# eigenkernel/eigenkernel

Measured on AMD Instinct MI355X. Metric: eigenpairs/s (full spectrum) + achieved fp64 TFLOP/s vs roofline, N=16384 GEP, higher is better.
Workload: dtype f64

## Files before the change

### eigenkernel_amd/csrc/ek_sb2st.hip

```cpp
#include "ek_common.h"
#include "ek_switch.h"

#include <cstdlib>
#include <type_traits>
#include <vector>

namespace ek {
namespace {

typedef double double4_t __attribute__((ext_vector_type(4)));

constexpr int SB = kBandW;
constexpr int LDAB = 2 * SB;
constexpr int DLD = SB + 1;

__device__ __forceinline__ double ld_sc1(const double *p) {
  return __longlong_as_double((long long)__hip_atomic_load((const unsigned long long *)p, __ATOMIC_RELAXED,
                                                           __HIP_MEMORY_SCOPE_AGENT));
}
__device__ __forceinline__ void st_sc1(double *p, double v) {
  __hip_atomic_store((unsigned long long *)p, (unsigned long long)__double_as_longlong(v), __ATOMIC_RELAXED,
                     __HIP_MEMORY_SCOPE_AGENT);
}
template <int CTRL>
__device__ __forceinline__ double dpp_mov(double v) {
  const int lo = __builtin_amdgcn_update_dpp(0, __double2loint(v), CTRL, 0xf, 0xf, false);
  const int hi = __builtin_amdgcn_update_dpp(0, __double2hiint(v), CTRL, 0xf, 0xf, false);
  return __hiloint2double(hi, lo);
}
template <int W>
__device__ __forceinline__ double group_sum(double v) {
  if (W >= 2) v += dpp_mov<0xB1>(v);
  if (W >= 4) v += dpp_mov<0x4E>(v);
  if (W >= 8) v += dpp_mov<0x141>(v);
  if (W >= 16) v += dpp_mov<0x140>(v);
  return v;
}
__device__ __forceinline__ double lane_value(double v, int l) {
  const int lo = __builtin_amdgcn_readlane(__double2loint(v), l);
  const int hi = __builtin_amdgcn_readlane(__double2hiint(v), l);
  return __hiloint2double(hi, lo);
}
template <int CTRL, int ROWMASK>
__device__ __forceinline__ double dpp_mov_rows(double v) {
  const int lo = __builtin_amdgcn_update_dpp(0, __double2loint(v), CTRL, ROWMASK, 0xf, false);
  const int hi = __builtin_amdgcn_update_dpp(0, __double2hiint(v), CTRL, ROWMASK, 0xf, false);
  return __hiloint2double(hi, lo);
}
__device__ __forceinline__ double wave_sum(double v) {
  v = group_sum<16>(v);
  v += dpp_mov_rows<0x142, 0xA>(v);
  v += dpp_mov_rows<0x143, 0xC>(v);
  return lane_value(v, 63);
}
__device__ __forceinline__ void wave_sync() {
  __builtin_amdgcn_s_waitcnt(0xc07f);
  __builtin_amdgcn_wave_barrier();
}

__global__ void pack_band_kernel(int n, const double *__restrict__ A, int lda, double *__restrict__ AB) {
  const int c = blockIdx.x;
  for (int d = threadIdx.x; d < LDAB; d += blockDim.x) {
    double v = 0.0;
    if (d <= SB && c + d < n) v = A[(size_t)(c + d) + (size_t)c * lda];
    AB[(size_t)d + (size_t)c * LDAB] = v;
  }
}
__global__ void unpack_de_kernel(int n, const double *__restrict__ AB, double *__restrict__ d, double *__restrict__ e) {
  const int c = blockIdx.x * blockDim.x + threadIdx.x;
  if (c >= n) return;
  d[c] = AB[(size_t)c * LDAB];
  if (c < n - 1) e[c] = AB[1 + (size_t)c * LDAB];
}

struct ChaseArgs {
  int n, nsweeps;
  double *AB;
  double *V2; int ldv2;
  double *tau2; int ldt;
  unsigned *prog;
  unsigned *ctl;
  double *mail; int kmax;
  int only_if_abandoned;
  const int *skip;
};

constexpr unsigned kSpinLimit = 1u << 22;

struct Reflector { double v, tau, beta; };

__device__ __forceinline__ Reflector reflector_of(double x, int lane) {
#pragma clang fp contract(off)
  const double ssq = wave_sum((lane >= 1) ? x * x : 0.0);
  const double alpha0 = lane_value(x, 0);
  Reflector r;
  r.beta = alpha0; r.tau = 0.0;
  double scale = 0.0;
  const double nrm2 = __builtin_fma(alpha0, alpha0, ssq);
  if (ssq != 0.0 && nrm2 > 1e-290) {
    r.beta = -copysign(sqrt(nrm2), alpha0);
    r.tau = (r.beta - alpha0) / r.beta;
    scale = 1.0 / (alpha0 - r.beta);
  }
  r.v = (lane == 0) ? 1.0 : x * scale;
  return r;
}
template <int CW>
__device__ __forceinline__ void task_partials(const double (&dd)[CW], const double (&bk)[CW], const double (&vc)[CW],
                                              double &pp, double &qq) {
#pragma clang fp contract(off)
  pp = 0.0; qq = 0.0;
#pragma unroll
  for (int j = 0; j < CW; ++j) { pp = __builtin_fma(dd[j], vc[j], pp); qq = __builtin_fma(bk[j], vc[j], qq); }
}
__device__ __forceinline__ double task_col0(double bk0, double tau, double qs, double vc0) {
#pragma clang fp contract(off)
  const double t = tau * qs;
  return __builtin_fma(-t, vc0, bk0);
}
__device__ __forceinline__ double task_w(double tau, double psum, double v_r) {
#pragma clang fp contract(off)
  const double p_r = tau * psum;
  const double dot = wave_sum(p_r * v_r);
  const double alpha = (-0.5 * tau) * dot;
  return __builtin_fma(alpha, v_r, p_r);
}
__device__ __forceinline__ double task_rank2(double d, double v_r, double w_c, double w_r, double v_c) {
#pragma clang fp contract(off)
  const double t1 = v_r * w_c, t2 = w_r * v_c;
  return d - (t1 + t2);
}
__device__ __forceinline__ double task_right(double b, double q_r, double v_c) {
#pragma clang fp contract(off)
  return __builtin_fma(-q_r, v_c, b);
}
template <int CW>
__device__ __forceinline__ void task_left(double (&bp)[CW], double vn_r, double tau_n, double *st, int lane, bool skip0) {
#pragma clang fp contract(off)
  constexpr int LPC = 64 / CW;
#pragma unroll
  for (int j = 0; j < CW; ++j) st[j * 65 + lane] = vn_r * bp[j];
  wave_sync();
  double tot_b;
  {
    const int j = lane / LPC, q = lane % LPC;
    const double *src = st + j * 65 + CW * q;
    double a0 = 0.0, a1 = 0.0;
#pragma unroll
    for (int l = 0; l < CW; l += 2) { a0 += src[l]; a1 += src[l + 1]; }
    tot_b = group_sum<LPC>(a0 + a1);
  }
  const double u = tau_n * vn_r;
#pragma unroll
  for (int j = 0; j < CW; ++j)
    if (!(skip0 && j == 0)) bp[j] = __builtin_fma(-u, lane_value(tot_b, j * LPC), bp[j]);
  wave_sync();
}

constexpr int MAILW = 72;
constexpr unsigned long long kMailEmpty = 0x7ff8dead0000beefull;

__device__ __forceinline__ bool mail_empty(double v) { return (unsigned long long)__double_as_longlong(v) == kMailEmpty; }

__global__ void mail_init_kernel(double *mail, int count) {
  const int i = blockIdx.x * blockDim.x + threadIdx.x;
  if (i < count) mail[i] = __longlong_as_double((long long)kMailEmpty);
}

template <int NW>
__global__ __launch_bounds__(64 * NW) void chase_kernel(ChaseArgs p) {
  constexpr int CW = SB / NW;
  __shared__ __attribute__((aligned(16))) double s_v[2][SB];
  __shared__ double s_p[NW][SB], s_q[NW][SB];
  __shared__ double s_t[NW][CW * 65];
  __shared__ double s_D[SB * DLD];
  __shared__ double s_tau[2];
  __shared__ int s_sweep, s_ok;
  const int t = threadIdx.x, lane = t & 63, wave = t >> 6;
  const int n = p.n;
  const int c0w = CW * wave;
  double *AB = p.AB;
  if (p.only_if_abandoned && !__hip_atomic_load(&p.ctl[3], __ATOMIC_RELAXED, __HIP_MEMORY_SCOPE_AGENT)) return;
  if (p.skip && (*p.skip & 0xff)) return;
  if (t == 0) s_ok = 1;
  auto give_up = [&]() { __hip_atomic_store(&p.ctl[1], 1u, __ATOMIC_RELAXED, __HIP_MEMORY_SCOPE_AGENT); };
  auto wait_word = [&](const unsigned *w, unsigned need) -> bool {
    unsigned spins = 0;
    while (__hip_atomic_load(w, __ATOMIC_RELAXED, __HIP_MEMORY_SCOPE_AGENT) < need) {
      __builtin_amdgcn_s_sleep(1);
      if ((++spins & 63u) == 0u &&
          (spins > kSpinLimit || __hip_atomic_load(&p.ctl[1], __ATOMIC_RELAXED, __HIP_MEMORY_SCOPE_AGENT)))
        return false;
    }
    return true;
  };
  auto put_reflector = [&](const Reflector &r, int L, int i0, int s, int k, double *sv, double *stau) {
    sv[lane] = r.v;
    if (lane == 0) { *stau = r.tau; p.tau2[(size_t)k + (size_t)s * p.ldt] = r.tau; }
    if (lane < L) p.V2[(size_t)(i0 + lane) + (size_t)s * p.ldv2] = r.v;
  };
  while (true) {
    __syncthreads();
    if (t == 0) s_sweep = (int)atomicAdd(&p.ctl[0], 1u);
    __syncthreads();
    const int s = s_sweep;
    if (s >= p.nsweeps) break;
    const int K = (n - 3 - s) / SB + 1;
    const int Kprev = (s > 0) ? (n - 2 - s) / SB + 1 : 0;
    const bool has_follower = s + 1 < p.nsweeps;
    for (int k = 0; k < K; ++k) {
      const int i0 = s + 1 + k * SB;
      const int L = (n - i0 < SB) ? n - i0 : SB;
      int L1 = n - i0 - SB; if (L1 > SB) L1 = SB; if (L1 < 0) L1 = 0;
      const bool lead = s > 0 && k + 1 < Kprev;
      double *mail = p.mail + ((size_t)((s - 1) & 3) * p.kmax + (k + 1)) * MAILW;
      if (t == 0 && s > 0) {
        if (!wait_word(&p.prog[s - 1], (unsigned)(k + 1 < Kprev ? k + 1 : Kprev))) { give_up(); s_ok = 0; }
      }
      __syncthreads();
      if (!s_ok) return;
      double dl[CW], bk[CW];
#pragma unroll
      for (int j = 0; j < CW; ++j) {
        const int c = c0w + j;
        dl[j] = (lane < L && c <= lane) ? ld_sc1(AB + (unsigned)((lane - c) + (i0 + c) * LDAB)) : 0.0;
        bk[j] = (lane < L1 && c < L) ? ld_sc1(AB + (unsigned)((SB + lane - c) + (i0 + c) * LDAB)) : 0.0;
      }
      double m_a = 0.0, m_b = 0.0;
      if (lead && wave == NW - 1) {
        m_a = ld_sc1(mail + ((lane < 63) ? lane + 1 : 64));
        if (lane == 63) m_b = ld_sc1(mail);
      }
      const int cur = k & 1;
      if (k == 0) {
        if (wave == 0) {
          const double x = (lane < L) ? ld_sc1(AB + (size_t)(1 + lane) + (size_t)s * LDAB) : 0.0;
          const Reflector r = reflector_of(x, lane);
          put_reflector(r, L, i0, s, k, s_v[cur], &s_tau[cur]);
          if (lane < L) st_sc1(AB + (size_t)(1 + lane) + (size_t)s * LDAB, (lane == 0) ? r.beta : 0.0);
        }
        __syncthreads();
      }
      const double tau = s_tau[cur];
      const double v_r = s_v[cur][lane];
      double vc[CW];
#pragma unroll
      for (int j = 0; j < CW; ++j) vc[j] = s_v[cur][c0w + j];
      if (lead && wave == NW - 1) {
        unsigned spins = 0;
        bool ok = true;
        while (__any(mail_empty(m_a) || (lane == 63 && mail_empty(m_b)))) {
          if ((++spins & 63u) == 0u &&
              (spins > kSpinLimit || __hip_atomic_load(&p.ctl[1], __ATOMIC_RELAXED, __HIP_MEMORY_SCOPE_AGENT))) {
            ok = false; break;
          }
          __builtin_amdgcn_s_sleep(1);
          if (mail_empty(m_a)) m_a = ld_sc1(mail + ((lane < 63) ? lane + 1 : 64));
          if (lane == 63 && mail_empty(m_b)) m_b = ld_sc1(mail);
        }
        if (!ok) { if (lane == 0) { give_up(); s_ok = 0; } }
        else {
          bk[CW - 1] = (lane < L1 && SB - 1 < L) ? m_a : 0.0;
          if (lane == 63 && SB - 1 < L) dl[CW - 1] = m_b;
          const double e = __longlong_as_double((long long)kMailEmpty);
          st_sc1(mail + ((lane < 63) ? lane + 1 : 64), e);
          if (lane == 63) st_sc1(mail, e);
        }
      }
#pragma unroll
      for (int j = 0; j < CW; ++j) {
        const int c = c0w + j;
        if (c <= lane) { s_D[lane * DLD + c] = dl[j]; s_D[c * DLD + lane] = dl[j]; }
      }
      __syncthreads();
      if (!s_ok) return;
      double dd[CW];
      {
        double pp, qq;
#pragma unroll
        for (int j = 0; j < CW; ++j) dd[j] = s_D[lane * DLD + c0w + j];
        task_partials<CW>(dd, bk, vc, pp, qq);
        s_p[wave][lane] = pp; s_q[wave][lane] = qq;
      }
      __syncthreads();
      if (wave == 0) {
        double qs = 0.0;
#pragma unroll
        for (int w = 0; w < NW; ++w) qs += s_q[w][lane];
        const double col0 = (L1 > 0) ? task_col0(bk[0], tau, qs, vc[0]) : 0.0;
        double b00 = col0;
        if (k + 1 < K) {
          const int i0n = i0 + SB;
          const Reflector r = reflector_of(col0, lane);
          put_reflector(r, L1, i0n, s, k + 1, s_v[cur ^ 1], &s_tau[cur ^ 1]);
          b00 = r.beta;
          if (lane < L1 && !(lane == 0 && k > 0 && has_follower))
            st_sc1(AB + (unsigned)((SB + lane) + i0 * LDAB), (lane == 0) ? r.beta : 0.0);
        }
        if (lane == 0 && k > 0 && has_follower)
          st_sc1(p.mail + ((size_t)(s & 3) * p.kmax + k) * MAILW + 64, b00);
      }
      double psum = 0.0;
#pragma unroll
      for (int w = 0; w < NW; ++w) psum += s_p[w][lane];
      const double w_r = task_w(tau, psum, v_r);
#pragma unroll
      for (int j = 0; j < CW; ++j) {
        const int c = c0w + j;
        dd[j] = task_rank2(dd[j], v_r, lane_value(w_r, c), w_r, vc[j]);
        if (c == 0 && k > 0 && has_follower)
          st_sc1(p.mail + ((size_t)(s & 3) * p.kmax + k) * MAILW + lane, dd[j]);
        if (c <= lane && lane < L && !(c == 0 && k > 0 && has_follower))
          st_sc1(AB + (unsigned)((lane - c) + (i0 + c) * LDAB), dd[j]);
      }
      double bp[CW];
#pragma unroll
      for (int j = 0; j < CW; ++j) bp[j] = 0.0;
      if (L1 > 0) {
        double qsum = 0.0;
#pragma unroll
        for (int w = 0; w < NW; ++w) qsum += s_q[w][lane];
        const double q_r = tau * qsum;
#pragma unroll
        for (int j = 0; j < CW; ++j) bp[j] = task_right(bk[j], q_r, vc[j]);
        if (k == K - 1) {
#pragma unroll
          for (int j = 0; j < CW; ++j) {
            const int c = c0w + j;
            if (lane < L1 && c < L && !(lane == 0 && c == 0 && k > 0 && has_follower))
              st_sc1(AB + (unsigned)((SB + lane - c) + (i0 + c) * LDAB), bp[j]);
          }
        }
      }
      if (k + 1 < K) {
        __syncthreads();
        task_left<CW>(bp, s_v[cur ^ 1][lane], s_tau[cur ^ 1], s_t[wave], lane, wave == 0);
#pragma unroll
        for (int j = 0; j < CW; ++j) {
          const int c = c0w + j;
          if (c > 0 && lane < L1)
            st_sc1(AB + (unsigned)((SB + lane - c) + (i0 + c) * LDAB), bp[j]);
        }
        asm volatile("s_waitcnt vmcnt(0)" ::: "memory");
        __syncthreads();
        if (t == 0) __hip_atomic_store(&p.prog[s], (unsigned)(k + 1), __ATOMIC_RELAXED, __HIP_MEMORY_SCOPE_AGENT);
      }
    }
    asm volatile("s_waitcnt vmcnt(0)" ::: "memory");
    __syncthreads();
    if (t == 0) __hip_atomic_store(&p.prog[s], (unsigned)K, __ATOMIC_RELAXED, __HIP_MEMORY_SCOPE_AGENT);
  }
}

constexpr int PMAILW = 80;
struct PosArgs {
  int n, K0;
  double *AB;
  double *V2; int ldv2;
  double *tau2; int ldt;
  double *fwd, *bwd;
  unsigned *retired;
  unsigned *ctl;
  unsigned census_spins;
  const int *skip;
  unsigned jitter;
};

template <int CTRL>
__device__ __forceinline__ double dpp_shift(double v) {
  const int lo = __builtin_amdgcn_update_dpp(__double2loint(v), __double2loint(v), CTRL, 0xf, 0xf, false);
  const int hi = __builtin_amdgcn_update_dpp(__double2hiint(v), __double2hiint(v), CTRL, 0xf, 0xf, false);
  return __hiloint2double(hi, lo);
}

__global__ __launch_bounds__(512) void chase_pos_kernel(PosArgs p) {
  constexpr int NW = 8, CW = SB / NW;
  __shared__ __attribute__((aligned(16))) double s_v[2][SB];
  __shared__ double s_p[NW][SB], s_q[NW][SB];
  __shared__ double s_t[NW][CW * 65];
  __shared__ double s_x[NW][SB], s_y[NW][SB], s_row[SB], s_b0[SB];
  __shared__ double s_tau[2], s_b00;
  __shared__ int s_ok;
  constexpr int RW = 1;
  const int t = threadIdx.x, lane = t & 63, wave = t >> 6;
  const int k = (int)blockIdx.x;
  if (k >= p.K0) return;
  if (p.skip && (*p.skip & 0xff)) return;
  const int n = p.n;
  const int c0w = CW * wave;
  double *AB = p.AB;
  unsigned *abandoned = &p.ctl[3];
  auto give_up = [&]() { __hip_atomic_store(abandoned, 1u, __ATOMIC_RELAXED, __HIP_MEMORY_SCOPE_AGENT); };
  if (t == 0) {
    int ok = 1;
    atomicAdd(&p.ctl[4], 1u);
    unsigned spins = 0;
    while (__hip_atomic_load(&p.ctl[4], __ATOMIC_RELAXED, __HIP_MEMORY_SCOPE_AGENT) < (unsigned)p.K0) {
      __builtin_amdgcn_s_sleep(8);
      if (++spins > p.census_spins || __hip_atomic_load(abandoned, __ATOMIC_RELAXED, __HIP_MEMORY_SCOPE_AGENT)) { ok = 0; break; }
    }
    if (!ok) give_up();
    s_ok = ok;
  }
  __syncthreads();
  if (!s_ok) return;
  auto take_line = [&](double *line, bool with65, double &a, double &b) -> bool {
    const bool l65 = with65 && lane == 0;
    a = ld_sc1(line + lane); b = l65 ? ld_sc1(line + 64) : 0.0;
    __builtin_amdgcn_s_sleep(2);
    double a2 = ld_sc1(line + lane), b2 = l65 ? ld_sc1(line + 64) : 0.0;
    unsigned spins = 0;
    while (__any(mail_empty(a) || (l65 && mail_empty(b)))) {
      if ((++spins & 63u) == 0u &&
          (spins > kSpinLimit || __hip_atomic_load(abandoned, __ATOMIC_RELAXED, __HIP_MEMORY_SCOPE_AGENT)))
        return false;
      a = a2; b = b2;
      a2 = ld_sc1(line + lane); b2 = l65 ? ld_sc1(line + 64) : 0.0;
    }
    const double e = __longlong_as_double((long long)kMailEmpty);
    st_sc1(line + lane, e);
    if (l65) st_sc1(line + 64, e);
    return true;
  };
  const int s_last = n - 3 - SB * k;
  double dd[CW], bk[CW];
  {
    const int i0 = 1 + SB * k;
    const int L = (n - i0 < SB) ? n - i0 : SB;
    int L1 = n - i0 - SB; if (L1 > SB) L1 = SB; if (L1 < 0) L1 = 0;
#pragma unroll
    for (int j = 0; j < CW; ++j) {
      const int c = c0w + j;
      const int hi = (lane > c) ? lane : c, lo = (lane > c) ? c : lane;
      dd[j] = (lane < L && c < L) ? AB[(size_t)(hi - lo) + (size_t)(i0 + lo) * LDAB] : 0.0;
      bk[j] = (lane < L1 && c < L) ? AB[(size_t)(SB + lane - c) + (size_t)(i0 + c) * LDAB] : 0.0;
    }
  }
  double xnext = 0.0;
  for (int s = 0; s <= s_last; ++s) {
    const int i0 = s + 1 + k * SB;
    const int L = (n - i0 < SB) ? n - i0 : SB;
    int L1 = n - i0 - SB; if (L1 > SB) L1 = SB; if (L1 < 0) L1 = 0;
    const int K = (n - 3 - s) / SB + 1;
    const int Kprev = (s > 0) ? (n - 2 - s) / SB + 1 : 0;
    const bool lead = s > 0 && k + 1 < Kprev;
    asm volatile("s_waitcnt vmcnt(0)" ::: "memory");
    if (p.jitter) {
      const unsigned h = ((unsigned)s * 2654435761u) ^ ((unsigned)k * 40503u * p.jitter);
      if (((h >> 9) & 15u) == 0u) for (unsigned q = 0; q < ((h >> 3) & 63u); ++q) __builtin_amdgcn_s_sleep(64);
    }
    if (wave == 0) {
      if (k == 0) {
        const double x = (s == 0) ? ((lane < L) ? AB[(size_t)(1 + lane)] : 0.0) : xnext;
        const Reflector r = reflector_of(x, lane);
        s_v[0][lane] = r.v;
        if (lane == 0) { s_tau[0] = r.tau; p.tau2[(size_t)s * p.ldt] = r.tau; AB[(size_t)1 + (size_t)s * LDAB] = r.beta; }
        if (lane < L) p.V2[(size_t)(i0 + lane) + (size_t)s * p.ldv2] = r.v;
      } else {
        double a, b;
        if (!take_line(p.fwd + ((size_t)k * 4 + (s & 3)) * PMAILW, false, a, b)) { if (lane == 0) { give_up(); s_ok = 0; } }
        s_v[0][lane] = (lane == 0) ? 1.0 : a;
        if (lane == 0) s_tau[0] = a;
      }
    }
    if (wave == NW - 1 && s > 0) {
      if (lead) {
        double a, b;
        if (!take_line(p.bwd + ((size_t)k * 4 + ((s - 1) & 3)) * PMAILW, true, a, b)) { if (lane == 0) { give_up(); s_ok = 0; } }
        const double up = dpp_shift<0x130>(a);
        const double beta = lane_value(b, 0), corner = lane_value(a, 0);
        const double col = (lane < 63) ? up : beta;
        bk[CW - 1] = (lane < L1 && SB - 1 < L) ? col : 0.0;
        if (lane == 63 && SB - 1 < L) dd[CW - 1] = corner;
      } else if (L == SB) {
        int ok = 1;
        if (lane == 0) {
          unsigned spins = 0;
          while (!__hip_atomic_load(&p.retired[k + 1], __ATOMIC_RELAXED, __HIP_MEMORY_SCOPE_AGENT)) {
            __builtin_amdgcn_s_sleep(1);
            if ((++spins & 63u) == 0u &&
                (spins > kSpinLimit || __hip_atomic_load(abandoned, __ATOMIC_RELAXED, __HIP_MEMORY_SCOPE_AGENT))) { ok = 0; break; }
          }
          if (!ok) { give_up(); s_ok = 0; }
        }
        wave_sync();
        const double corner = ld_sc1(AB + (size_t)(i0 + SB - 1) * LDAB);
        if (lane == 63) dd[CW - 1] = corner;
      }
    }
    __syncthreads();
    if (!s_ok) return;
    const double tau = s_tau[0];
    const double v_r = s_v[0][lane];
    double vc[CW];
#pragma unroll
    for (int j = 0; j < CW; ++j) vc[j] = s_v[0][c0w + j];
    {
      double pp, qq;
      task_partials<CW>(dd, bk, vc, pp, qq);
      s_p[wave][lane] = pp; s_q[wave][lane] = qq;
      if (wave == 0) s_b0[lane] = bk[0];
    }
    __syncthreads();
    if (wave == RW) {
      double qs = 0.0;
#pragma unroll
      for (int w = 0; w < NW; ++w) qs += s_q[w][lane];
      const double col0 = (L1 > 0) ? task_col0(s_b0[lane], tau, qs, s_v[0][0]) : 0.0;
      double b00 = col0;
      if (k + 1 < K) {
        const Reflector r = reflector_of(col0, lane);
        double *line = p.fwd + ((size_t)(k + 1) * 4 + (s & 3)) * PMAILW;
        st_sc1(line + lane, (lane == 0) ? r.tau : r.v);
        s_v[1][lane] = r.v;
        if (lane == 0) { s_tau[1] = r.tau; p.tau2[(size_t)(k + 1) + (size_t)s * p.ldt] = r.tau; }
        if (lane < L1) p.V2[(size_t)(i0 + SB + lane) + (size_t)s * p.ldv2] = r.v;
        b00 = r.beta;
      }
      if (lane == 0) {
        if (k > 0) st_sc1(p.bwd + ((size_t)(k - 1) * 4 + (s & 3)) * PMAILW + 64, b00);
        else s_b00 = b00;
      }
    }
    double psum = 0.0;
#pragma unroll
    for (int w = 0; w < NW; ++w) psum += s_p[w][lane];
    const double w_r = task_w(tau, psum, v_r);
    if (wave == 0) {
      dd[0] = task_rank2(dd[0], v_r, lane_value(w_r, 0), w_r, vc[0]);
      if (k > 0) st_sc1(p.bwd + ((size_t)(k - 1) * 4 + (s & 3)) * PMAILW + lane, dd[0]);
      else if (lane == 0) AB[(size_t)(s + 1) * LDAB] = dd[0];
    }
#pragma unroll
    for (int j = 0; j < CW; ++j)
      if (!(wave == 0 && j == 0)) dd[j] = task_rank2(dd[j], v_r, lane_value(w_r, c0w + j), w_r, vc[j]);
    double bp[CW];
    {
      double qsum = 0.0;
#pragma unroll
      for (int w = 0; w < NW; ++w) qsum += s_q[w][lane];
      const double q_r = tau * qsum;
#pragma unroll
      for (int j = 0; j < CW; ++j) bp[j] = (L1 > 0) ? task_right(bk[j], q_r, vc[j]) : 0.0;
    }
    if (k + 1 < K) {
      __syncthreads();
      task_left<CW>(bp, s_v[1][lane], s_tau[1], s_t[wave], lane, wave == 0);
    }
    if (s == s_last) break;
    if (lane == 0) {
#pragma unroll
      for (int j = 0; j < CW; ++j) s_row[c0w + j] = bp[j];
    }
    s_x[wave][lane] = dd[0]; s_y[wave][lane] = bp[0];
    __syncthreads();
    if (k == 0 && wave == 0) {
      const double up = dpp_shift<0x130>(dd[0]);
      xnext = (lane < 63) ? up : s_b00;
    }
#pragma unroll
    for (int j = 0; j + 1 < CW; ++j) { dd[j] = dd[j + 1]; bk[j] = bp[j + 1]; }
    dd[CW - 1] = (wave + 1 < NW) ? s_x[(wave + 1) & (NW - 1)][lane] : 0.0;
    bk[CW - 1] = (wave + 1 < NW) ? s_y[(wave + 1) & (NW - 1)][lane] : 0.0;
#pragma unroll
    for (int j = 0; j < CW; ++j) {
      const double brow0 = lane_value(bk[j], 0);
      const double du = dpp_shift<0x130>(dd[j]), bu = dpp_shift<0x130>(bk[j]);
      dd[j] = (lane == 63) ? brow0 : du;
      bk[j] = (lane == 63) ? 0.0 : bu;
    }
    if (wave == NW - 1) dd[CW - 1] = (lane < 63) ? s_row[lane + 1] : 0.0;
  }
  if (wave == 0) {
    if (lane == 1) {
      st_sc1(AB + (size_t)(n - 1) * LDAB, dd[1]);
      if (k == 0) st_sc1(AB + (size_t)1 + (size_t)(n - 2) * LDAB, dd[0]);
    }
    asm volatile("s_waitcnt vmcnt(0)" ::: "memory");
    if (lane == 0) __hip_atomic_store(&p.retired[k], 1u, __ATOMIC_RELAXED, __HIP_MEMORY_SCOPE_AGENT);
  }
}

__global__ void set_word_kernel(unsigned *p, unsigned v) { *p = v; }

__global__ void repack_band_kernel(int n, const double *__restrict__ AB0, double *__restrict__ AB, const unsigned *ctl) {
  if (!ctl[3]) return;
  const int c = blockIdx.x;
  for (int d = threadIdx.x; d < LDAB; d += blockDim.x) AB[(size_t)d + (size_t)c * LDAB] = AB0[(size_t)d + (size_t)c * LDAB];
}

constexpr int QG = 32;
constexpr int QR = QG + SB;
constexpr int QVLD = QG + 1;
constexpr int QREC = 2 * QR * QG;

struct Q2Geom {
  int n, nsweeps, nS, kmax;
  const unsigned *offS;
};
__host__ __device__ inline int q2_first_sweep(int S) { return S * QG - 1; }
__host__ __device__ inline int q2_groups_of_block(int n, int S) {
  int s0 = q2_first_sweep(S); if (s0 < 0) s0 = 0;
  return (s0 <= n - 3) ? (n - 3 - s0) / SB + 1 : 0;
}

__device__ __forceinline__ double q2_v_entry(const Q2Geom &g, const double *__restrict__ V2, int ldv2, int S, int k,
                                             int rr, int i) {
  const int s = q2_first_sweep(S) + i, o = S * QG + k * SB, row = o + rr;
  if (s < 0 || s >= g.nsweeps || rr < i || rr >= i + SB || row >= g.n) return 0.0;
  if (s + 1 + k * SB > g.n - 2) return 0.0;
  return V2[(size_t)row + (size_t)s * ldv2];
}

__global__ __launch_bounds__(256) void q2_tfactor_kernel(Q2Geom g, const double *__restrict__ V2, int ldv2,
                                                         const double *__restrict__ tau2, int ldt,
                                                         double *__restrict__ Rec) {
  __shared__ double sV[QR * QVLD];
  __shared__ double sG[QG * QVLD];
  __shared__ double sT[QG * QVLD];
  __shared__ double s_tau[QG];
  const int S = blockIdx.y, k = blockIdx.x, t = threadIdx.x, lane = t & 63, wave = t >> 6;
  const int l15 = lane & 15, l4 = lane >> 4;
  if (k >= q2_groups_of_block(g.n, S)) return;
  double *rec = Rec + ((size_t)g.offS[S] + k) * QREC;
  for (int idx = t; idx < QR * QG; idx += 256) {
    const int rr = idx % QR, i = idx / QR;
    const double v = q2_v_entry(g, V2, ldv2, S, k, rr, i);
    sV[rr * QVLD + i] = v;
    rec[rr * QG + i] = v;
  }
  for (int idx = t; idx < QG * QVLD; idx += 256) sT[idx] = 0.0;
  if (t < QG) {
    const int s = q2_first_sweep(S) + t;
    const bool exists = s >= 0 && s < g.nsweeps && s + 1 + k * SB <= g.n - 2;
    s_tau[t] = exists ? tau2[(size_t)k + (size_t)s * ldt] : 0.0;
  }
  __syncthreads();
  {
    const int ti = wave >> 1, tj = wave & 1;
    double4_t acc = (double4_t){0.0, 0.0, 0.0, 0.0};
    for (int kk = 0; kk < QR; kk += 4) {
      const double x = sV[(kk + l4) * QVLD + 16 * ti + l15];
      const double y = sV[(kk + l4) * QVLD + 16 * tj + l15];
      acc = __builtin_amdgcn_mfma_f64_16x16x4f64(x, y, acc, 0, 0, 0);
    }
#pragma unroll
    for (int r = 0; r < 4; ++r) sG[(16 * ti + l4 + 4 * r) * QVLD + 16 * tj + l15] = acc[r];
  }
  __syncthreads();
  if (wave == 0) {
    for (int i = 0; i < QG; ++i) {
      const double ti = s_tau[i];
      if (lane < i) {
        double a0 = 0.0, a1 = 0.0;
        int l = lane;
        for (; l + 1 < i; l += 2) {
          a0 += sT[lane * QVLD + l] * sG[l * QVLD + i];
          a1 += sT[lane * QVLD + l + 1] * sG[(l + 1) * QVLD + i];
        }
        if (l < i) a0 += sT[lane * QVLD + l] * sG[l * QVLD + i];
        sT[lane * QVLD + i] = -ti * (a0 + a1);
      } else if (lane == i) sT[i * QVLD + i] = ti;
      wave_sync();
    }
  }
  __syncthreads();
  for (int tile = wave; tile < 12; tile += 4) {
    const int ti = tile >> 1, tj = tile & 1;
    double4_t acc = (double4_t){0.0, 0.0, 0.0, 0.0};
#pragma unroll
    for (int kk = 0; kk < QG; kk += 4) {
      const double x = sV[(16 * ti + l15) * QVLD + kk + l4];
      const double y = sT[(kk + l4) * QVLD + 16 * tj + l15];
      acc = __builtin_amdgcn_mfma_f64_16x16x4f64(x, y, acc, 0, 0, 0);
    }
#pragma unroll
    for (int r = 0; r < 4; ++r) rec[QR * QG + (16 * ti + l4 + 4 * r) * QG + 16 * tj + l15] = -acc[r];
  }
}

constexpr int QNC = 64;
constexpr int QSTLD = 34;
constexpr int QVS = QG, QTS = QG + 2;
constexpr int QOPSZ = QR * QVS + QR * QTS;
constexpr unsigned kQ2Done = 0x7fffffffu;

struct Q2ApplyArgs {
  Q2Geom g;
  const double *Rec;
  double *Z; int ldz; int ncols;
  int nslab, npass, npair;
  unsigned *prog;
  unsigned *ctl;
};

typedef double d2_t __attribute__((ext_vector_type(2)));
__device__ __forceinline__ void st_sc1_x2(double *p, double a, double b) {
  d2_t v = {a, b};
  asm volatile("global_store_dwordx4 %0, %1, off sc1" :: "v"(p), "v"(v) : "memory");
}

#ifndef Q2_PF
#define Q2_PF 1
#endif
#ifndef Q2_PUTV0
#define Q2_PUTV0 24
#define Q2_PUTVS 4
#endif
template <int NBLK>
__global__ __launch_bounds__(256, 2) void q2_apply_nb_kernel(Q2ApplyArgs p) {
  constexpr int WT = 2 * NBLK + 4;
  extern __shared__ __attribute__((aligned(16))) double q2smem[];
  double *sOp = q2smem;
  __shared__ int s_pass, s_ok;
  const int t = threadIdx.x, lane = t & 63, wave = t >> 6, l15 = lane & 15, l4 = lane >> 4;
  double *st = q2smem + QOPSZ + wave * 16 * QSTLD;
  const int n = p.g.n;
  const double *sV = sOp, *sVT = sOp + QR * QVS;
  while (true) {
    __syncthreads();
    if (t == 0) s_pass = (int)atomicAdd(&p.ctl[2], 1u);
    __syncthreads();
    const int pass = __builtin_amdgcn_readfirstlane(s_pass);
    if (pass >= p.npass) break;
    const int bundle = p.npair - 1 - pass / p.nslab, slab = pass % p.nslab;
    const int S = NBLK * bundle;
    auto ks_of = [&](int b) -> int { return (S + b < p.g.nS) ? q2_groups_of_block(n, S + b) : 0; };
    auto off_of = [&](int b) -> unsigned {
      return (S + b < p.g.nS) ? (unsigned)__builtin_amdgcn_readfirstlane((int)p.g.offS[S + b]) : 0u;
    };
    const int KS0 = ks_of(0), KS1 = NBLK > 1 ? ks_of(1) : 0, KS2 = NBLK > 2 ? ks_of(2) : 0, KS3 = NBLK > 3 ? ks_of(3) : 0;
    const unsigned of0 = off_of(0), of1 = NBLK > 1 ? off_of(1) : 0u, of2 = NBLK > 2 ? off_of(2) : 0u, of3 = NBLK > 3 ? off_of(3) : 0u;
    auto KSb = [&](int b) -> int { return b == 0 ? KS0 : (b == 1 ? KS1 : (b == 2 ? KS2 : KS3)); };
    const int KS = KS0;
    const int colw = slab * QNC + 16 * wave;
    const unsigned *pprog = (bundle + 1 < p.npair) ? p.prog + (size_t)(pass - p.nslab) : nullptr;
    unsigned *myprog = p.prog + pass;
    if (KS <= 0) { if (t == 0) __hip_atomic_store(myprog, kQ2Done, __ATOMIC_RELAXED, __HIP_MEMORY_SCOPE_AGENT); continue; }
    const int o0 = S * QG;
    auto wait_for = [&](unsigned need) -> bool {
      if (!pprog) return true;
      unsigned spins = 0;
      while (__hip_atomic_load(pprog, __ATOMIC_RELAXED, __HIP_MEMORY_SCOPE_AGENT) < need) {
        __builtin_amdgcn_s_sleep(2);
        if ((++spins & 63u) == 0u &&
            (spins > kSpinLimit || __hip_atomic_load(&p.ctl[1], __ATOMIC_RELAXED, __HIP_MEMORY_SCOPE_AGENT)))
          return false;
      }
      return true;
    };
    double4_t w[WT];
    static_assert(QR * QG == 6 * 256 * 2, "a half record is six 16-byte pairs per thread");
    constexpr int HALF = QR * QG / 2;
    double zreg[16];
    d2_t oreg[12];
    const int obase_v = (t >> 4) * QVS + ((2 * (t & 15) + 16 * ((t >> 4) & 1)) & 31);
    const int obase_t = (t >> 4) * QTS + 2 * (t & 15);
    const int vsw = 16 * (l4 & 1);
    auto rec_of = [&](int b, int k) -> const d2_t * {
      const unsigned o = b == 0 ? of0 : (b == 1 ? of1 : (b == 2 ? of2 : of3));
      return reinterpret_cast<const d2_t *>(p.Rec + ((size_t)o + k) * QREC) + t;
    };
    auto fetch_v = [&](const d2_t *rec) {
#pragma unroll
      for (int q = 0; q < 6; ++q) oreg[q] = rec[256 * q];
    };
    auto fetch_t = [&](const d2_t *rec) {
#pragma unroll
      for (int q = 0; q < 6; ++q) oreg[6 + q] = rec[HALF + 256 * q];
    };
    auto put_v = [&](int q) { *reinterpret_cast<d2_t *>(sOp + obase_v + q * 16 * QVS) = oreg[q]; };
    auto put_t = [&](int q) { *reinterpret_cast<d2_t *>(sOp + QR * QVS + obase_t + q * 16 * QTS) = oreg[6 + q]; };
    const bool cols_in = colw + 16 <= p.ncols;
    auto fetch_rows = [&](int row0) {
      const int row = row0 + lane;
      const double *src = p.Z + (size_t)row + (size_t)colw * p.ldz;
      if (cols_in && row0 + SB <= n) {
#pragma unroll
        for (int c = 0; c < 16; ++c) zreg[c] = ld_sc1(src + (size_t)c * p.ldz);
      } else {
#pragma unroll
        for (int c = 0; c < 16; ++c)
          zreg[c] = (row < n && colw + c < p.ncols) ? ld_sc1(src + (size_t)c * p.ldz) : 0.0;
      }
    };
    auto half_to_tiles = [&](int h, double4_t &ta, double4_t &tb) {
      if ((lane >> 5) == h) {
#pragma unroll
        for (int c = 0; c < 16; ++c) st[c * QSTLD + (lane & 31)] = zreg[c];
      }
      wave_sync();
#pragma unroll
      for (int r = 0; r < 4; ++r) { ta[r] = st[l15 * QSTLD + l4 + 4 * r]; tb[r] = st[l15 * QSTLD + 16 + l4 + 4 * r]; }
      wave_sync();
    };
    auto tiles_to_rows = [&](int row0, const double4_t &ta, const double4_t &tb) {
#pragma unroll
      for (int r = 0; r < 4; ++r) { st[l15 * QSTLD + l4 + 4 * r] = ta[r]; st[l15 * QSTLD + 16 + l4 + 4 * r] = tb[r]; }
      wave_sync();
      {
        const int pr = lane & 15, cg = lane >> 4;
        const int row = row0 + 2 * pr;
        double *dst0 = p.Z + (size_t)row + (size_t)(colw + 4 * cg) * p.ldz;
        if (cols_in && row0 + 32 <= n) {
#pragma unroll
          for (int q = 0; q < 4; ++q) {
            const int c = 4 * cg + q;
            st_sc1_x2(dst0 + (size_t)q * p.ldz, st[c * QSTLD + 2 * pr], st[c * QSTLD + 2 * pr + 1]);
          }
        } else {
#pragma unroll
          for (int q = 0; q < 4; ++q) {
            const int c = 4 * cg + q;
            if (colw + c < p.ncols) {
              const double a = st[c * QSTLD + 2 * pr], b = st[c * QSTLD + 2 * pr + 1];
              if (row + 1 < n) st_sc1_x2(dst0 + (size_t)q * p.ldz, a, b);
              else if (row < n) st_sc1(dst0 + (size_t)q * p.ldz, a);
            }
          }
        }
      }
      wave_sync();
    };
    auto apply_group = [&](auto off_c, const d2_t *nrec, int row_next) {
      constexpr int OFF = decltype(off_c)::value;
      constexpr int PF = Q2_PF;
      double4_t w1[2];
      w1[0] = (double4_t){0.0, 0.0, 0.0, 0.0}; w1[1] = (double4_t){0.0, 0.0, 0.0, 0.0};
      {
        double pa[PF + 1][2];
        auto ld1 = [&](int sidx, int slot) {
          const double *vrow = sV + (16 * (sidx >> 2) + 4 * (sidx & 3) + l4) * QVS + l15;
          pa[slot][0] = vrow[vsw]; pa[slot][1] = vrow[16 - vsw];
        };
#pragma unroll
        for (int q = 0; q < PF; ++q) ld1(q, q);
#pragma unroll
        for (int sidx = 0; sidx < 24; ++sidx) {
          if (sidx + PF < 24) ld1(sidx + PF, (sidx + PF) % (PF + 1));
          if (sidx < 12 && (sidx & 1) == 0) put_t(sidx >> 1);
          if (sidx == 12) {
            fetch_v(nrec);
            if (row_next >= 0) fetch_rows(row_next);
          }
          const int tile = sidx >> 2, r = sidx & 3;
          const double y = w[tile + OFF][r];
          if (tile < 5) w1[0] = __builtin_amdgcn_mfma_f64_16x16x4f64(pa[sidx % (PF + 1)][0], y, w1[0], 0, 0, 0);
          if (tile > 0) w1[1] = __builtin_amdgcn_mfma_f64_16x16x4f64(pa[sidx % (PF + 1)][1], y, w1[1], 0, 0, 0);
        }
      }
      __syncthreads();
      fetch_t(nrec);
      {
        double px[PF + 1];
        auto seq_tile = [](int q) { return 2 * (q >> 4) + (q & 1); };
        auto seq_kk = [](int q) { return 4 * ((q & 15) >> 1); };
        auto seq_ok = [&](int q) { return !(seq_tile(q) == 5 && seq_kk(q) < 16); };
        auto ld2 = [&](int q, int slot) {
          if (seq_ok(q)) px[slot] = sVT[(16 * seq_tile(q) + l15) * QTS + l4 + seq_kk(q)];
        };
#pragma unroll
        for (int q = 0; q < PF; ++q) ld2(q, q);
#pragma unroll
        for (int q = 0; q < 48; ++q) {
          if (q + PF < 48) ld2(q + PF, (q + PF) % (PF + 1));
          if (q >= Q2_PUTV0 && q < Q2_PUTV0 + 6 * Q2_PUTVS && (q - Q2_PUTV0) % Q2_PUTVS == 0) put_v((q - Q2_PUTV0) / Q2_PUTVS);
          if (seq_ok(q)) {
            const int tile = seq_tile(q), kk = seq_kk(q);
            w[tile + OFF] = __builtin_amdgcn_mfma_f64_16x16x4f64(px[q % (PF + 1)], w1[kk >> 4][(kk & 15) >> 2], w[tile + OFF], 0, 0, 0);
          }
        }
      }
    };
    auto first_block = [&](int k) -> int {
      int b = 0;
#pragma unroll
      for (int q = 1; q < NBLK; ++q) if (k < KSb(q)) b = q;
      return b;
    };
    auto next_group = [&](int k, int b) -> const d2_t * {
      int nb = -1, nk = k;
#pragma unroll
      for (int q = NBLK - 1; q >= 0; --q) if (q < b && nb < 0 && k < KSb(q)) nb = q;
      if (nb < 0) { nk = k + 1; if (nk < KS) nb = first_block(nk); }
      if (nb < 0) { nb = b; nk = k; }
      return rec_of(nb, nk);
    };
    if (t == 0) s_ok = wait_for(1u) ? 1 : 0;
    __syncthreads();
    if (!s_ok) { if (t == 0) __hip_atomic_store(&p.ctl[1], 1u, __ATOMIC_RELAXED, __HIP_MEMORY_SCOPE_AGENT); return; }
#pragma unroll
    for (int c = 0; c < WT / 4; ++c) {
      fetch_rows(o0 + 64 * c);
      half_to_tiles(0, w[4 * c], w[4 * c + 1]);
      half_to_tiles(1, w[4 * c + 2], w[4 * c + 3]);
    }
    if (WT % 4) {
      fetch_rows(o0 + 64 * (WT / 4));
      half_to_tiles(0, w[WT - 2], w[WT - 1]);
    }
    fetch_v(rec_of(first_block(0), 0));
    fetch_t(rec_of(first_block(0), 0));
#pragma unroll
    for (int q = 0; q < 6; ++q) put_v(q);
    unsigned early = 0;
    for (int k = 0; k < KS; ++k) {
      if (t == 0) {
        const unsigned need = (unsigned)(k + 2);
        s_ok = (!pprog || early >= need || wait_for(need)) ? 1 : 0;
      }
      __syncthreads();
      if (!s_ok) { if (t == 0) __hip_atomic_store(&p.ctl[1], 1u, __ATOMIC_RELAXED, __HIP_MEMORY_SCOPE_AGENT); return; }
      if (t == 0 && k > 1) __hip_atomic_store(myprog, (unsigned)(k - 1), __ATOMIC_RELAXED, __HIP_MEMORY_SCOPE_AGENT);
      const int bfirst = first_block(k);
      auto do_group = [&](auto b_c) {
        constexpr int B = decltype(b_c)::value;
        if (k >= KSb(B)) return;
        if (B == bfirst && t == 0 && pprog) early = __hip_atomic_load(pprog, __ATOMIC_RELAXED, __HIP_MEMORY_SCOPE_AGENT);
        apply_group(std::integral_constant<int, 2 * B>(), next_group(k, B),
                    (B == bfirst && k + 1 < KS) ? o0 + 64 * (k + 1) + 16 * (WT - 4) : -1);
        if (B > 0) __syncthreads();
      };
      if constexpr (NBLK >= 4) do_group(std::integral_constant<int, 3>());
      if constexpr (NBLK >= 3) do_group(std::integral_constant<int, 2>());
      if constexpr (NBLK >= 2) do_group(std::integral_constant<int, 1>());
      do_group(std::integral_constant<int, 0>());
      asm volatile("s_waitcnt vmcnt(0)" ::: "memory");
      tiles_to_rows(o0 + 64 * k, w[0], w[1]);
      tiles_to_rows(o0 + 64 * k + 32, w[2], w[3]);
#pragma unroll
      for (int i = 0; i + 4 < WT; ++i) w[i] = w[i + 4];
      if (k + 1 < KS) {
        half_to_tiles(0, w[WT - 4], w[WT - 3]);
        half_to_tiles(1, w[WT - 2], w[WT - 1]);
      } else {
#pragma unroll
        for (int i = 0; i + 4 < WT; i += 2) tiles_to_rows(o0 + 64 * (k + 1) + 16 * i, w[i], w[i + 1]);
      }
    }
    asm volatile("s_waitcnt vmcnt(0)" ::: "memory");
    __syncthreads();
    if (t == 0) __hip_atomic_store(myprog, kQ2Done, __ATOMIC_RELAXED, __HIP_MEMORY_SCOPE_AGENT);
  }
}

__global__ void forward_abort_kernel(const unsigned *ctl, int *flag) { if (ctl[1]) atomicOr(flag, 4); }
__global__ void q2_offsets_kernel(int n, int nS, unsigned *offS) {
  if (threadIdx.x == 0 && blockIdx.x == 0) {
    unsigned o = 0;
    for (int S = 0; S < nS; ++S) { offS[S] = o; o += (unsigned)q2_groups_of_block(n, S); }
    offS[nS] = o;
  }
}

inline size_t al256(size_t b) { return (b + 255) & ~(size_t)255; }

struct Layout {
  int nsweeps, nS, kmax, ldt;
  size_t off_ab0, off_ab, off_tau, off_prog, off_mail, off_pmail, off_retired, off_ctl, off_T, off_qprog, off_offs, total;
  size_t nrec;
  explicit Layout(int n, bool with_records = true) {
    nsweeps = n > 2 ? n - 2 : 0;
    nS = ceil_div((nsweeps > 0 ? nsweeps : 1) + 1, QG);
    kmax = q2_groups_of_block(n, 0); if (kmax < 1) kmax = 1;
    ldt = kmax + 1;
    size_t o = 0;
    off_ab0 = o; o += al256((size_t)LDAB * (round_up(n + 1, 128)) * 8);
    off_ab = o; o += al256((size_t)LDAB * (n + 1) * 8);
    off_tau = o; o += al256((size_t)ldt * (nsweeps + 1) * 8);
    off_prog = o; o += al256((size_t)(nsweeps + 1) * 4);
    off_mail = o; o += al256((size_t)4 * (kmax + 1) * MAILW * 8);
    off_pmail = o; o += al256((size_t)2 * 4 * (kmax + 2) * PMAILW * 8);
    off_retired = o; o += al256((size_t)(kmax + 2) * 4);
    off_ctl = o; o += 256;
    nrec = 0;
    for (int S = 0; S < nS; ++S) nrec += (size_t)q2_groups_of_block(n, S);
    off_T = o; o += with_records ? al256((nrec + 1) * QREC * 8) : 0;
    off_qprog = o; o += al256((size_t)nS * ceil_div(n, QNC) * 4);
    off_offs = o; o += al256((size_t)(nS + 1) * 4);
    total = o;
  }
};

int pos_capacity() {
  static int cap = -1;
  if (cap < 0) {
    int per_cu = 0, dev = 0;
    hipDeviceProp_t pr;
    if (hipGetDevice(&dev) != hipSuccess || hipGetDeviceProperties(&pr, dev) != hipSuccess ||
        hipOccupancyMaxActiveBlocksPerMultiprocessor(&per_cu, chase_pos_kernel, 512, 0) != hipSuccess)
      cap = 0;
    else {
      if (per_cu > 2) per_cu = 2;
      cap = per_cu * pr.multiProcessorCount;
    }
  }
  return cap;
}

}

size_t sb2st_work_bytes(int n, bool with_records) { return Layout(n, with_records).total; }
size_t sb2st_record_bytes(int n) { return al256((Layout(n).nrec + 1) * QREC * 8); }
void sb2st_debug_view(int n, void *work, const double **tau2, int *ldt, const unsigned **ctl) {
  const Layout L(n, false);
  *tau2 = (const double *)((char *)work + L.off_tau);
  *ldt = L.ldt;
  *ctl = (const unsigned *)((char *)work + L.off_ctl);
}

double *sb2st_band(void *work, int n) { return (double *)((char *)work + Layout(n, false).off_ab0); }
void pack_band(hipStream_t s, int n, const double *A, int lda, double *AB) {
  if (n <= 0) return;
  hipLaunchKernelGGL(pack_band_kernel, dim3(n), dim3(LDAB), 0, s, n, A, lda, AB);
}

void sb2st_lower(hipStream_t s, int n, const double *A, int lda, double *d, double *e, double *V2, int ldv2,
                 int *d_flag, void *work, bool band_packed, int chase_mode) {
  if (n <= 0) return;
  const Layout L(n, false);
  char *w = (char *)work;
  double *AB0 = (double *)(w + L.off_ab0);
  double *AB = (double *)(w + L.off_ab), *tau2 = (double *)(w + L.off_tau);
  unsigned *prog = (unsigned *)(w + L.off_prog), *ctl = (unsigned *)(w + L.off_ctl);
  double *mail = (double *)(w + L.off_mail), *pmail = (double *)(w + L.off_pmail);
  unsigned *retired = (unsigned *)(w + L.off_retired);
  const int nmail = 4 * (L.kmax + 1) * MAILW, npmail = 2 * 4 * (L.kmax + 2) * PMAILW;
  if (!band_packed) hipLaunchKernelGGL(pack_band_kernel, dim3(n), dim3(LDAB), 0, s, n, A, lda, AB0);
  (void)hipMemcpyAsync(AB, AB0, (size_t)LDAB * n * 8, hipMemcpyDeviceToDevice, s);
  (void)hipMemsetAsync(tau2, 0, (size_t)L.ldt * (L.nsweeps + 1) * 8, s);
  (void)hipMemsetAsync(prog, 0, (size_t)(L.nsweeps + 1) * 4 + 0, s);
  (void)hipMemsetAsync(ctl, 0, 256, s);
  if (L.nsweeps > 0) {
    int mode = 2;
    if (switch_int(kSwChase) > 0) mode = switch_int(kSwChase);
    if (chase_mode > 0) mode = chase_mode;
    const int K0 = (n - 3) / SB + 1;
    const bool pos = mode == 2 && K0 <= pos_capacity() && !switch_text(kSwChaseWgs);
    kprof_begin(s, kProfChase);
    if (pos) {
      hipLaunchKernelGGL(mail_init_kernel, dim3(ceil_div(npmail, 256)), dim3(256), 0, s, pmail, npmail);
      (void)hipMemsetAsync(retired, 0, (size_t)(L.kmax + 2) * 4, s);
      hipLaunchKernelGGL(set_word_kernel, dim3(1), dim3(1), 0, s, retired + K0, 1u);
      const unsigned census = (unsigned)switch_int(kSwCensusSpins);
      PosArgs a{n, K0, AB, V2, ldv2, tau2, L.ldt, pmail, pmail + (size_t)4 * (L.kmax + 2) * PMAILW, retired, ctl, census, d_flag,
                (unsigned)switch_int(kSwChaseJitter)};
      hipLaunchKernelGGL(chase_pos_kernel, dim3(K0), dim3(512), 0, s, a);
      hipLaunchKernelGGL(repack_band_kernel, dim3(n), dim3(LDAB), 0, s, n, AB0, AB, ctl);
    }
    hipLaunchKernelGGL(mail_init_kernel, dim3(ceil_div(nmail, 256)), dim3(256), 0, s, mail, nmail);
    ChaseArgs c{n, L.nsweeps, AB, V2, ldv2, tau2, L.ldt, prog, ctl, mail, L.kmax + 1, pos ? 1 : 0, d_flag};
    int nwg = n / SB + 8;
    if (nwg > 256) nwg = 256;
    if (nwg > L.nsweeps) nwg = L.nsweeps;
    if (switch_int(kSwChaseWgs) > 0) nwg = switch_int(kSwChaseWgs);
    hipLaunchKernelGGL(chase_kernel<8>, dim3(nwg), dim3(512), 0, s, c);
    kprof_end(s, kProfChase);
  }
  hipLaunchKernelGGL(unpack_de_kernel, dim3(ceil_div(n, 256)), dim3(256), 0, s, n, AB, d, e);
  hipLaunchKernelGGL(forward_abort_kernel, dim3(1), dim3(1), 0, s, ctl, d_flag);
}

void sb2st_apply_q2(hipStream_t s, int n, int ncols, const double *V2, int ldv2, double *Z, int ldz, int *d_flag,
                    void *work, double *records) {
  if (n <= 2 || ncols <= 0) return;
  const Layout L(n, records == nullptr);
  char *w = (char *)work;
  const double *tau2 = (const double *)(w + L.off_tau);
  double *Rec = records ? records : (double *)(w + L.off_T);
  unsigned *ctl = (unsigned *)(w + L.off_ctl), *qprog = (unsigned *)(w + L.off_qprog);
  unsigned *offS = (unsigned *)(w + L.off_offs);
  hipLaunchKernelGGL(q2_offsets_kernel, dim3(1), dim3(64), 0, s, n, L.nS, offS);
  Q2Geom g{n, L.nsweeps, L.nS, L.kmax, offS};
  hipLaunchKernelGGL(q2_tfactor_kernel, dim3(L.kmax, L.nS), dim3(256), 0, s, g, V2, ldv2, tau2, L.ldt, Rec);
  constexpr size_t lds = (size_t)(QOPSZ + 4 * 16 * QSTLD) * sizeof(double);
  static bool attr = false;
  if (!attr) {
    (void)hipFuncSetAttribute((const void *)q2_apply_nb_kernel<2>, hipFuncAttributeMaxDynamicSharedMemorySize, (int)lds);
    (void)hipFuncSetAttribute((const void *)q2_apply_nb_kernel<3>, hipFuncAttributeMaxDynamicSharedMemorySize, (int)lds);
    (void)hipFuncSetAttribute((const void *)q2_apply_nb_kernel<4>, hipFuncAttributeMaxDynamicSharedMemorySize, (int)lds);
    attr = true;
  }
  int nblk = (n >= 8192) ? 4 : 3;
  { const int v = switch_int(kSwQ2Nblk); if (v >= 2 && v <= 4) nblk = v; }
  const int per = nblk;
  const int npair = ceil_div(L.nS, per);
  const size_t qcap = al256((size_t)L.nS * ceil_div(n, QNC) * 4) / 4;
  const int slabs_max = (int)(qcap / (size_t)npair);
  if (ceil_div(ncols, QNC) > slabs_max) {
    const int piece = slabs_max * QNC;
    for (int c0 = 0; c0 < ncols; c0 += piece)
      sb2st_apply_q2(s, n, (ncols - c0 < piece) ? ncols - c0 : piece, V2, ldv2, Z + (size_t)c0 * ldz, ldz, d_flag, work, records);
    return;
  }
  const int nslab = ceil_div(ncols, QNC), npass = npair * nslab;
  (void)hipMemsetAsync(qprog, 0, (size_t)npass * 4, s);
  (void)hipMemsetAsync(ctl + 2, 0, 4, s);
  Q2ApplyArgs a{g, Rec, Z, ldz, ncols, nslab, npass, npair, qprog, ctl};
  const int nwg = npass < 512 ? npass : 512;
  kprof_begin(s, kProfQ2Apply);
  if (nblk == 3) hipLaunchKernelGGL(q2_apply_nb_kernel<3>, dim3(nwg), dim3(256), lds, s, a);
  else if (nblk == 4) hipLaunchKernelGGL(q2_apply_nb_kernel<4>, dim3(nwg), dim3(256), lds, s, a);
  else hipLaunchKernelGGL(q2_apply_nb_kernel<2>, dim3(nwg), dim3(256), lds, s, a);
  kprof_end(s, kProfQ2Apply);
  if (d_flag) hipLaunchKernelGGL(forward_abort_kernel, dim3(1), dim3(1), 0, s, ctl, d_flag);
}

}
```

Baseline: 20180.

## Pack Q2 V/T records to skip structurally zero triangles

Introduces a compact record layout for the Q2 back-transform that stores only the nonzero band parts of the V and T images (5+5 16-byte slots per thread instead of 6+6), with a constexpr slot map shared by producer and consumer. The tfactor kernel writes the packed record via LDS staging, and the apply kernel fetches and scatters fewer pairs into pre-zeroed LDS images. This cuts global record traffic and register use per group, at the cost of more irregular LDS offsets and extra syncs in the tfactor kernel.

```diff
diff --git a/eigenkernel_amd/csrc/ek_q2_record.h b/eigenkernel_amd/csrc/ek_q2_record.h
--- /dev/null
+++ b/eigenkernel_amd/csrc/ek_q2_record.h
@@ -0,0 +1,72 @@
+#pragma once
+
+#if defined(__HIPCC__) || defined(__CUDACC__)
+#define EK_Q2REC_HD __host__ __device__
+#else
+#define EK_Q2REC_HD
+#endif
+
+namespace ek {
+namespace q2rec {
+
+constexpr int kRows = 96, kCols = 32;
+constexpr int kThreads = 256;
+constexpr int kVLoads = 5, kTLoads = 5, kLoads = kVLoads + kTLoads;
+constexpr int kSlots = kThreads * kLoads;
+constexpr int kRecDoubles = 2 * kSlots;
+constexpr int kRecBytes = 16 * kSlots;
+constexpr int kVLd = 32, kTLd = 34;
+
+struct Slot {
+  int image;
+  int row;
+  int pair;
+  bool pad;
+};
+
+EK_Q2REC_HD constexpr bool v_nonzero(int rr, int i) { return i <= rr && rr < i + 64; }
+EK_Q2REC_HD constexpr bool t_nonzero(int rr, int j) { return rr < 64 || (rr <= 94 && j >= rr - 63); }
+EK_Q2REC_HD constexpr bool nonzero(int image, int rr, int col) { return image ? t_nonzero(rr, col) : v_nonzero(rr, col); }
+
+EK_Q2REC_HD constexpr Slot lower_triangle(int image, int u, int c) {
+  const int sa = (u + 1) >> 1;
+  return c >= sa ? Slot{image, 64 + u, c, false} : Slot{image, 95 - u, 16 - sa + c, false};
+}
+
+EK_Q2REC_HD constexpr Slot slot_of_thread(int q, int t) {
+  const int u = t >> 4, c = t & 15;
+  if (q < 2) return Slot{0, 32 + u + 16 * q, c, false};
+  if (q == 2) return lower_triangle(0, u, c);
+  if (q == 3) {
+    if (u == 15) return Slot{0, 30, c, false};
+    const int na = (u >> 1) + 1;
+    return c < na ? Slot{0, u, c, false} : Slot{0, 29 - u, c - na, false};
+  }
+  if (q == 4) {
+    if (u == 0) return Slot{0, 31, c, false};
+    const int v = u - 1, na = (v >> 1) + 1;
+    return c >= na ? Slot{0, v, c, true} : Slot{0, 29 - v, 16 - na + c, true};
+  }
+  if (q < 9) return Slot{1, u + 16 * (q - kVLoads), c, false};
+  return lower_triangle(1, u, c);
+}
+
+EK_Q2REC_HD constexpr Slot slot_of(int s) { return slot_of_thread(s / kThreads, s % kThreads); }
+
+EK_Q2REC_HD constexpr int v_lds_offset(int row, int pair) { return row * kVLd + ((2 * pair + 16 * (row & 1)) & 31); }
+EK_Q2REC_HD constexpr int t_lds_offset(int row, int pair) { return row * kTLd + 2 * pair; }
+EK_Q2REC_HD constexpr int lds_offset(const Slot &s) { return s.image ? t_lds_offset(s.row, s.pair) : v_lds_offset(s.row, s.pair); }
+
+EK_Q2REC_HD constexpr bool dense_slots_are_16_rows_apart() {
+  for (int t = 0; t < kThreads; ++t) {
+    if (lds_offset(slot_of(kThreads + t)) != lds_offset(slot_of(t)) + 16 * kVLd) return false;
+    for (int q = 1; q < 4; ++q)
+      if (lds_offset(slot_of((kVLoads + q) * kThreads + t)) != lds_offset(slot_of(kVLoads * kThreads + t)) + q * 16 * kTLd)
+        return false;
+  }
+  return true;
+}
+static_assert(dense_slots_are_16_rows_apart(), "the reader's strides");
+
+}
+}
diff --git a/eigenkernel_amd/csrc/ek_sb2st.hip b/eigenkernel_amd/csrc/ek_sb2st.hip
--- a/eigenkernel_amd/csrc/ek_sb2st.hip
+++ b/eigenkernel_amd/csrc/ek_sb2st.hip
@@ -1,5 +1,6 @@
 #include "ek_common.h"
 #include "ek_switch.h"
+#include "ek_q2_record.h"
 
 #include <cstdlib>
 #include <type_traits>
@@ -592,7 +593,10 @@
 constexpr int QG = 32;
 constexpr int QR = QG + SB;
 constexpr int QVLD = QG + 1;
-constexpr int QREC = 2 * QR * QG;
+constexpr int QREC = q2rec::kRecDoubles;
+static_assert(q2rec::kRows == QR && q2rec::kCols == QG && q2rec::kThreads == 256, "ek_q2_record.h describes these images");
+
+typedef double d2_t __attribute__((ext_vector_type(2)));
 
 struct Q2Geom {
   int n, nsweeps, nS, kmax;
@@ -627,7 +631,6 @@
     const int rr = idx % QR, i = idx / QR;
     const double v = q2_v_entry(g, V2, ldv2, S, k, rr, i);
     sV[rr * QVLD + i] = v;
-    rec[rr * QG + i] = v;
   }
   for (int idx = t; idx < QG * QVLD; idx += 256) sT[idx] = 0.0;
   if (t < QG) {
@@ -636,6 +639,13 @@
     s_tau[t] = exists ? tau2[(size_t)k + (size_t)s * ldt] : 0.0;
   }
   __syncthreads();
+  d2_t *rec2 = reinterpret_cast<d2_t *>(rec);
+#pragma unroll
+  for (int q = 0; q < q2rec::kVLoads; ++q) {
+    const q2rec::Slot sl = q2rec::slot_of(256 * q + t);
+    const double *src = sV + sl.row * QVLD + 2 * sl.pair;
+    rec2[256 * q + t] = sl.pad ? (d2_t){0.0, 0.0} : (d2_t){src[0], src[1]};
+  }
   {
     const int ti = wave >> 1, tj = wave & 1;
     double4_t acc = (double4_t){0.0, 0.0, 0.0, 0.0};
@@ -665,17 +675,31 @@
     }
   }
   __syncthreads();
-  for (int tile = wave; tile < 12; tile += 4) {
-    const int ti = tile >> 1, tj = tile & 1;
-    double4_t acc = (double4_t){0.0, 0.0, 0.0, 0.0};
+  double4_t acc[3];
+#pragma unroll
+  for (int w3 = 0; w3 < 3; ++w3) {
+    const int tile = wave + 4 * w3, ti = tile >> 1, tj = tile & 1;
+    acc[w3] = (double4_t){0.0, 0.0, 0.0, 0.0};
 #pragma unroll
     for (int kk = 0; kk < QG; kk += 4) {
       const double x = sV[(16 * ti + l15) * QVLD + kk + l4];
       const double y = sT[(kk + l4) * QVLD + 16 * tj + l15];
-      acc = __builtin_amdgcn_mfma_f64_16x16x4f64(x, y, acc, 0, 0, 0);
-    }
-#pragma unroll
-    for (int r = 0; r < 4; ++r) rec[QR * QG + (16 * ti + l4 + 4 * r) * QG + 16 * tj + l15] = -acc[r];
+      acc[w3] = __builtin_amdgcn_mfma_f64_16x16x4f64(x, y, acc[w3], 0, 0, 0);
+    }
+  }
+  __syncthreads();
+#pragma unroll
+  for (int w3 = 0; w3 < 3; ++w3) {
+    const int tile = wave + 4 * w3, ti = tile >> 1, tj = tile & 1;
+#pragma unroll
+    for (int r = 0; r < 4; ++r) sV[(16 * ti + l4 + 4 * r) * QVLD + 16 * tj + l15] = -acc[w3][r];
+  }
+  __syncthreads();
+#pragma unroll
+  for (int q = q2rec::kVLoads; q < q2rec::kLoads; ++q) {
+    const q2rec::Slot sl = q2rec::slot_of(256 * q + t);
+    const double *src = sV + sl.row * QVLD + 2 * sl.pair;
+    rec2[256 * q + t] = (d2_t){src[0], src[1]};
   }
 }
 
@@ -694,7 +718,6 @@
   unsigned *ctl;
 };
 
-typedef double d2_t __attribute__((ext_vector_type(2)));
 __device__ __forceinline__ void st_sc1_x2(double *p, double a, double b) {
   d2_t v = {a, b};
   asm volatile("global_store_dwordx4 %0, %1, off sc1" :: "v"(p), "v"(v) : "memory");
@@ -717,6 +740,7 @@
   double *st = q2smem + QOPSZ + wave * 16 * QSTLD;
   const int n = p.g.n;
   const double *sV = sOp, *sVT = sOp + QR * QVS;
+  for (int idx = t; idx < QOPSZ; idx += 256) sOp[idx] = idx < QR * QVS ? 0.0 : -0.0;
   while (true) {
     __syncthreads();
     if (t == 0) s_pass = (int)atomicAdd(&p.ctl[2], 1u);
@@ -750,12 +774,13 @@
       return true;
     };
     double4_t w[WT];
-    static_assert(QR * QG == 6 * 256 * 2, "a half record is six 16-byte pairs per thread");
-    constexpr int HALF = QR * QG / 2;
+    constexpr int NV = q2rec::kVLoads, NT = q2rec::kTLoads;
+    static_assert(QVS == q2rec::kVLd && QTS == q2rec::kTLd, "ek_q2_record.h places the slots in these images");
     double zreg[16];
-    d2_t oreg[12];
-    const int obase_v = (t >> 4) * QVS + ((2 * (t & 15) + 16 * ((t >> 4) & 1)) & 31);
-    const int obase_t = (t >> 4) * QTS + 2 * (t & 15);
+    d2_t oreg[NV + NT];
+    auto slot_off = [&](int q) -> int { return q2rec::lds_offset(q2rec::slot_of_thread(q, t)); };
+    const int obase_v = slot_off(0), ov2 = slot_off(2), ov3 = slot_off(3), ov4 = slot_off(4);
+    const int obase_t = slot_off(NV), ot4 = slot_off(NV + 4);
     const int vsw = 16 * (l4 & 1);
     auto rec_of = [&](int b, int k) -> const d2_t * {
       const unsigned o = b == 0 ? of0 : (b == 1 ? of1 : (b == 2 ? of2 : of3));
@@ -763,14 +788,20 @@
     };
     auto fetch_v = [&](const d2_t *rec) {
 #pragma unroll
-      for (int q = 0; q < 6; ++q) oreg[q] = rec[256 * q];
+      for (int q = 0; q < NV; ++q) oreg[q] = rec[256 * q];
     };
     auto fetch_t = [&](const d2_t *rec) {
 #pragma unroll
-      for (int q = 0; q < 6; ++q) oreg[6 + q] = rec[HALF + 256 * q];
-    };
-    auto put_v = [&](int q) { *reinterpret_cast<d2_t *>(sOp + obase_v + q * 16 * QVS) = oreg[q]; };
-    auto put_t = [&](int q) { *reinterpret_cast<d2_t *>(sOp + QR * QVS + obase_t + q * 16 * QTS) = oreg[6 + q]; };
+      for (int q = 0; q < NT; ++q) oreg[NV + q] = rec[256 * (NV + q)];
+    };
+    auto put_v = [&](int q) {
+      const int o = q < 2 ? obase_v + q * 16 * QVS : (q == 2 ? ov2 : (q == 3 ? ov3 : ov4));
+      *reinterpret_cast<d2_t *>(sOp + o) = oreg[q];
+    };
+    auto put_t = [&](int q) {
+      const int o = q < 4 ? obase_t + q * 16 * QTS : ot4;
+      *reinterpret_cast<d2_t *>(sOp + QR * QVS + o) = oreg[NV + q];
+    };
     const bool cols_in = colw + 16 <= p.ncols;
     auto fetch_rows = [&](int row0) {
       const int row = row0 + lane;
@@ -838,7 +869,7 @@
 #pragma unroll
         for (int sidx = 0; sidx < 24; ++sidx) {
           if (sidx + PF < 24) ld1(sidx + PF, (sidx + PF) % (PF + 1));
-          if (sidx < 12 && (sidx & 1) == 0) put_t(sidx >> 1);
+          if (sidx < 2 * NT && (sidx & 1) == 0) put_t(sidx >> 1);
           if (sidx == 12) {
             fetch_v(nrec);
             if (row_next >= 0) fetch_rows(row_next);
@@ -864,7 +895,7 @@
 #pragma unroll
         for (int q = 0; q < 48; ++q) {
           if (q + PF < 48) ld2(q + PF, (q + PF) % (PF + 1));
-          if (q >= Q2_PUTV0 && q < Q2_PUTV0 + 6 * Q2_PUTVS && (q - Q2_PUTV0) % Q2_PUTVS == 0) put_v((q - Q2_PUTV0) / Q2_PUTVS);
+          if (q >= Q2_PUTV0 && q < Q2_PUTV0 + NV * Q2_PUTVS && (q - Q2_PUTV0) % Q2_PUTVS == 0) put_v((q - Q2_PUTV0) / Q2_PUTVS);
           if (seq_ok(q)) {
             const int tile = seq_tile(q), kk = seq_kk(q);
             w[tile + OFF] = __builtin_amdgcn_mfma_f64_16x16x4f64(px[q % (PF + 1)], w1[kk >> 4][(kk & 15) >> 2], w[tile + OFF], 0, 0, 0);
@@ -902,7 +933,7 @@
     fetch_v(rec_of(first_block(0), 0));
     fetch_t(rec_of(first_block(0), 0));
 #pragma unroll
-    for (int q = 0; q < 6; ++q) put_v(q);
+    for (int q = 0; q < NV; ++q) put_v(q);
     unsigned early = 0;
     for (int k = 0; k < KS; ++k) {
       if (t == 0) {
```

After: 20280, median of 6. Within noise of the previous version (+0.5%).
